# OkDoky/mpc_ros

Measured on AMD Instinct MI355X. Metric: NMPC solves/sec (whole node), N=20 diff-drive, at 1/2/4/8 MI355X, higher is better.
Workload: dtype f64

## Files before the change

### mpc_ros_amd/csrc/mpcg_wide_kern.h

```cpp
#ifndef MPCG_WIDE_KERN_H
#define MPCG_WIDE_KERN_H
#include <hip/hip_runtime.h>

#include "mpcg_internal.h"
#include "mpcg_pp.h"
#include "wave_dev.h"
#include "wide_core.h"
#include "wide_plan.h"

namespace mpcg {


struct WideArgs {
    IpmParams P;
    int64_t B;
    const int32_t* order;
    const double* state;
    const double* coeffs;
    double* u0;
    double* traj;
    int32_t* status;
    double* obj;
    int32_t* iters;
    int32_t* diag;
// ... 70 lines not shown
template <class Solver>
__device__ __forceinline__ void write_out(const WideArgs& a, Solver& S, int64_t p, int parked);
template <bool VHOLD = false>
__device__ __forceinline__ PPRow pp_load_row(const double* pparams, int64_t p) {
    typedef const double __attribute__((address_space(4))) cdouble;
    const cdouble* row = (const cdouble*)(pparams + p * MPCG_PP_FIELDS);
    PPRow r;
#pragma unroll
    for (int j = 0; j < MPCG_PP_FIELDS; ++j) {
        r.f[j] = row[j];
        if constexpr (VHOLD) asm("" : "+v"(r.f[j]));
    }
    return r;
}
#ifndef MPCG_PP_ROW_SGPR
#define MPCG_PP_ROW_SGPR 0
#endif
__device__ __forceinline__ void pp_invalid_out(const WideArgs& a, int64_t p) {
    const int t = threadIdx.x;
    if (t == 0) {
        a.u0[p * 2 + 0] = 0.0;
        a.u0[p * 2 + 1] = 0.0;
        if (a.status) a.status[p] = IPM_INTERNAL_ERROR;
        if (a.iters) a.iters[p] = 0;
        if (a.obj) a.obj[p] = __builtin_nan("");
    }
    if (a.diag && t < 4) a.diag[p * 4 + t] = 0;
    if (a.traj)
        for (int k = t; k < 3 * a.P.N; k += 64) a.traj[p * 3 * a.P.N + k] = 0.0;
    if (a.sol)
        for (int64_t e = t; e < a.sol_stride; e += 64) a.sol[p * a.sol_stride + e] = 0.0;
}

template <int MODEL, bool SPLIT, class T, int NB, bool DEFOPT, bool WARM, bool PP = false>
__device__ __forceinline__ void solve_body(const WideArgs& a, const double* pparams = nullptr) {
    if ((int64_t)blockIdx.x >= a.B) return;
    const int64_t p = a.order ? (int64_t)a.order[blockIdx.x] : (int64_t)blockIdx.x;
    check_index_quiet(p, a.n_prob);
    const int t = threadIdx.x;
    IpmProblem<T> pr;
#pragma unroll
    for (int j = 0; j < 6; ++j) pr.init[j] = (T)a.state[p * 6 + j];
#pragma unroll
    for (int j = 0; j < 4; ++j) pr.c[j] = (T)a.coeffs[p * 4 + j];
    DevWave wv;
    wv.t = t;
    IpmParams Pk = a.P;
    if constexpr (DEFOPT) ipopt_default_options(Pk);
    if (blockIdx.x == 0 && t == 0) atomicExch(a.started, 1);
    if constexpr (PP) {
        const PPRow row = pp_load_row<!MPCG_PP_ROW_SGPR>(pparams, p);
        if (!pp_row_ok(row.f, MODEL)) {
            pp_invalid_out(a, p);
            block_done(a.done);
            return;
        }
        pp_row_apply(row.f, Pk);
    }
    const int slot = claim_slot(a.slot_flags, a.nslots, a.nxcc, (int64_t)blockIdx.x);
    check_index_quiet(slot, a.nslots);
    typedef WideSolver<DevWave, MODEL, SPLIT, T, NB> Solver;
    Solver S(Pk, pr, wv, (T*)a.slots + (int64_t)slot * a.slot_elems);
    if constexpr (WARM) {
        const float* h = a.handoff + p * a.handoff_stride;
        if (__builtin_amdgcn_readfirstlane(h[0] != 0.0f ? 1 : 0))
            S.init_warm(h);
        else
            S.init();
        S.run();
    } else {
        S.solve();
    }
    if constexpr (sizeof(T) == 4) {
        if (a.handoff) {
            S.handoff_out(a.handoff + p * a.handoff_stride);
            release_slot(a.slot_flags, slot);
            block_done(a.done);
            return;
        }
    }
    if (S.status == Solver::NEED_RESTO) {
        int e = 0;
        if (t == 0) e = atomicAdd(a.park_count, 1);
        e = __builtin_amdgcn_readfirstlane(__shfl(e, 0, 64));
        if (e < a.park_cap) {
            check_index_quiet(e, a.park_cap);
            S.park((T*)a.park + (int64_t)e * a.park_stride, p);
            if (t == 0) a.park_idx[e] = p;
            __builtin_amdgcn_fence(__ATOMIC_RELEASE, "agent");
            __builtin_amdgcn_wave_barrier();
            if (t == 0) atomicExch(&a.park_ready[e], 1);
            release_slot(a.slot_flags, slot);
            block_done(a.done);
            return;
        }
        if (t == 0) {
            const int o = atomicAdd(a.ovf_count, 1);
            check_index_quiet(o, a.B);
            atomicExch((unsigned long long*)&a.ovf_idx[o], (unsigned long long)p);
        }
        release_slot(a.slot_flags, slot);
        block_done(a.done);
        return;
    }
    write_out(a, S, p, 0);
    release_slot(a.slot_flags, slot);
    block_done(a.done);
}

template <int MODEL, bool SPLIT, class T, int NB, bool DEFOPT = false, int WPE = 2>
__global__ void __launch_bounds__(64) __attribute__((amdgpu_waves_per_eu(WPE, WPE))) k_solve_wide(WideArgs a) {
    solve_body<MODEL, SPLIT, T, NB, DEFOPT, false>(a);
}
template <int MODEL, bool SPLIT, class T, int NB, bool DEFOPT = false, int WPE = 2>
__global__ void __launch_bounds__(64) __attribute__((amdgpu_waves_per_eu(WPE, WPE))) k_warm_wide(WideArgs a) {
    solve_body<MODEL, SPLIT, T, NB, DEFOPT, true>(a);
}

template <int MODEL, bool SPLIT, class T, int NB, bool DEFOPT = false, int WPE = 2>
__global__ void __launch_bounds__(64) __attribute__((amdgpu_waves_per_eu(WPE, WPE)))
k_solve_wide_pp(WideArgs a, const double* pparams) {
    solve_body<MODEL, SPLIT, T, NB, DEFOPT, false, true>(a, pparams);
}

template <class Solver>
__device__ __forceinline__ void write_out(const WideArgs& a, Solver& S, int64_t p, int parked) {
    const int t = threadIdx.x;
    if (a.diag && t == 0) {
        if (a.handoff && sizeof(typename Solver::T) == 8) parked = a.handoff[p * a.handoff_stride] != 0.0f ? 4 : 3;
        a.diag[p * 4 + 0] = S.n_resto;
        a.diag[p * 4 + 1] = S.n_fover;
        a.diag[p * 4 + 2] = parked;
        a.diag[p * 4 + 3] = S.nf_peak;
#ifdef MPCG_DEBUG_MU
        a.diag[p * 4 + 1] = (int)(-100.0 * log10((double)S.mu));
        a.diag[p * 4 + 3] = (int)(-100.0 * log10((double)S.compl0 + 1e-300));
#endif
    }
    const double o = (double)S.objective_out();
    const int N = a.P.N;
    if (t == 0) {
        a.u0[p * 2 + 0] = (double)S.x_ctrl(0, 0);
        a.u0[p * 2 + 1] = (double)S.x_ctrl(1, 0);
        if (a.status) a.status[p] = S.status;
        if (a.iters) a.iters[p] = S.iter;
// ... 69 lines not shown
                continue;
            }
            if ((int64_t)d >= a.B) break;
            const uint64_t now = wall_clock64();
            if (d == 0 && now - t_start > (uint64_t)200000 &&
                __hip_atomic_load(a.started, __ATOMIC_RELAXED, __HIP_MEMORY_SCOPE_AGENT) == 0)
                break;
            if (d != last_done) {
                last_done = d;
                t0 = now;
            } else if (now - t0 > (uint64_t)2000000000) {
                break;
            }
            __builtin_amdgcn_s_sleep(32);
        }
        if (o >= 0) {
            for (;;) {
                p = (int64_t)__hip_atomic_load((unsigned long long*)&a.ovf_idx[o], __ATOMIC_ACQUIRE,
                                               __HIP_MEMORY_SCOPE_AGENT);
                if (p >= 0) break;
                __builtin_amdgcn_s_sleep(8);
            }
        }
    }
    const int lo = __builtin_amdgcn_readfirstlane(__shfl((int)(p & 0xffffffff), 0, 64));
    const int hi = __builtin_amdgcn_readfirstlane(__shfl((int)(p >> 32), 0, 64));
    return (int64_t)(((uint64_t)(uint32_t)hi << 32) | (uint32_t)lo);
}

template <int MODEL, bool SPLIT, class T, int NB>
__global__ void __launch_bounds__(64) __attribute__((amdgpu_waves_per_eu(1, 1))) k_resume_wide(WideArgs a) {
    const int t = threadIdx.x;
    const WideLayout Lw(a.P.N, a.P.filter_cap, MODEL);
    typedef WideSolver<DevWave, MODEL, SPLIT, T, NB> Solver;
    for (;;) {
        int64_t p;
        T* ent;
        if (a.phase == 0) {
            const int e = take_parked(a);
            if (e < 0) return;
            check_index("parked entry", e, a.park_cap);
            p = a.park_idx[e];
            check_index("parked problem", p, a.n_prob);
            ent = (T*)a.park + (int64_t)e * a.park_stride;
        } else {
            p = take_overflow(a);
            if (p < 0) return;
            check_index("overflow problem", p, a.n_prob);
            check_index("overflow worker's park entry", (int64_t)a.ent0 + blockIdx.x, a.park_cap);
            ent = (T*)a.park + (int64_t)(a.ent0 + blockIdx.x) * a.park_stride;
        }
        IpmProblem<T> pr;
#pragma unroll
        for (int j = 0; j < 6; ++j) pr.init[j] = (T)a.state[p * 6 + j];
#pragma unroll
        for (int j = 0; j < 4; ++j) pr.c[j] = (T)a.coeffs[p * 4 + j];
        DevWave wv;
        wv.t = t;
        Solver S(a.P, pr, wv, ent + Solver::PARK_SCALARS + Lw.total());
        if (a.phase == 0) {
            if (!S.park_entry_ok(ent, p)) index_fault("parked entry's tag / counts: problem", p, a.n_prob);
            S.unpark(ent);
        } else {
            if (a.handoff && a.handoff[p * a.handoff_stride] != 0.0f)
                S.init_warm(a.handoff + p * a.handoff_stride);
            else
                S.init();
            S.run();
        }
        S.finish_resto();
        write_out(a, S, p, a.phase == 0 ? 1 : a.ovf_mark);
    }
}
template <int MODEL, bool SPLIT, class T, int NB>
__global__ void __launch_bounds__(64) __attribute__((amdgpu_waves_per_eu(1, 1)))
k_resume_wide_pp(WideArgs a, const double* pparams) {
    const int t = threadIdx.x;
    const WideLayout Lw(a.P.N, a.P.filter_cap, MODEL);
    typedef WideSolver<DevWave, MODEL, SPLIT, T, NB> Solver;
    for (;;) {
        int64_t p;
        T* ent;
        if (a.phase == 0) {
            const int e = take_parked(a);
            if (e < 0) return;
            check_index("parked entry", e, a.park_cap);
            p = a.park_idx[e];
            check_index("parked problem", p, a.n_prob);
            ent = (T*)a.park + (int64_t)e * a.park_stride;
        } else {
            p = take_overflow(a);
            if (p < 0) return;
            check_index("overflow problem", p, a.n_prob);
            check_index("overflow worker's park entry", (int64_t)a.ent0 + blockIdx.x, a.park_cap);
            ent = (T*)a.park + (int64_t)(a.ent0 + blockIdx.x) * a.park_stride;
        }
        IpmProblem<T> pr;
#pragma unroll
        for (int j = 0; j < 6; ++j) pr.init[j] = (T)a.state[p * 6 + j];
#pragma unroll
        for (int j = 0; j < 4; ++j) pr.c[j] = (T)a.coeffs[p * 4 + j];
        DevWave wv;
        wv.t = t;
        IpmParams Pk = a.P;
        const PPRow row = pp_load_row(pparams, p);
        pp_row_apply(row.f, Pk);
        Solver S(Pk, pr, wv, ent + Solver::PARK_SCALARS + Lw.total());
        if (a.phase == 0) {
            if (!S.park_entry_ok(ent, p)) index_fault("parked entry's tag / counts: problem", p, a.n_prob);
            S.unpark(ent);
        } else {
            S.init();
// ... 43 lines not shown
```

### mpc_ros_amd/csrc/wide_core.h

```cpp
#ifndef MPCG_WIDE_CORE_H
#define MPCG_WIDE_CORE_H

#include "ipm_core.h"

#ifndef MPCG_FUSE
#define MPCG_FUSE 3
#endif

namespace mpcg {

template <class T>
MPCG_HD T opaque(T v) {
#if defined(__HIP_DEVICE_COMPILE__)
    asm volatile("" : "+v"(v));
#endif
    return v;
}

struct WideLayout {
    int N, cap, SS;
    int KL;
    MPCG_HD WideLayout(int N_, int cap_, int model, int kl = -1)
        : N(N_), cap(cap_), SS(model == 1 ? 42 : 38), KL(kl >= 0 ? kl : (model == 1 || N_ > 32 ? 0 : KS)) {}
    static constexpr int WS = 10, YS = 6, KS = 18;
    static constexpr int RS = 34, RZL = 8, RZU = 16, RDW = 24;
    static constexpr int SA = 0;
    static constexpr int SDT = 7;
    static constexpr int SD = 8;
    static constexpr int SQD = 14;
    static constexpr int SQV = 22;
    static constexpr int SCV = 30;
    static constexpr int SZERO = 35, SONE = 36, SMONE = 37;
    static constexpr int KF = 16;
    static constexpr int STW = 38, STV = 39, SHVD = 40;
    MPCG_HD int W(int k) const { return RS * k; }
    MPCG_HD int ZL(int k) const { return RS * k + RZL; }
    MPCG_HD int ZU(int k) const { return RS * k + RZU; }
    MPCG_HD int DW(int k) const { return RS * k + RDW; }
    MPCG_HD int Y(int k) const { return RS * N + YS * k; }
// ... 25 lines not shown
    static constexpr int XM = 48;
    static constexpr int XMN = 84;
    static constexpr int XMV = 120;
    static constexpr int XE = 126;
    static constexpr int XRX = 132, XRP = 140, XRN = 146, XRC = 152;
    static constexpr int XSX = 158, XSP = 166, XSN = 172, XSY = 178, XSC = 184;
    static constexpr int XS = 190;
    static constexpr int XW = 72;
    MPCG_HD int SP_DUMP() const { return spill(); }
    MPCG_HD int SP_EXT() const { return spill() + total(); }
    MPCG_HD int SP_XSP() const { return SP_EXT() + XS * N; }
    MPCG_HD int SP_FLTR() const { return SP_XSP() + XW * N; }
    MPCG_HD int slot() const { return SP_FLTR() + 2 * FX; }
    static constexpr int PARK_SCALARS = 32, HANDOFF_HEAD = 4;
    MPCG_HD int park() const { return PARK_SCALARS + total() + slot(); }
    MPCG_HD static int handoff(int N_) { return HANDOFF_HEAD + 30 * N_; }
};

MPCG_HD int64_t solution_elems(int N) { return 3 * (int64_t)(8 * N - 2) + 6 * (int64_t)N; }

template <class T>
struct RestoIn {
    T mu, tau, theta, prim_inf, ref_phi, ref_theta, sf;
    int nf, iter;
};
struct RestoOut {
    int status;
    int iter;
    int fover;
};
template <class WV, int MODEL, class T, int NB>
MPCG_NOINLINE RestoOut resto_phase(const IpmParams& P, IpmProblem<T> pr, WV wv, T* ws, RestoIn<T> in);

template <class WV, int MODEL = 0, bool SPLIT = false, class TT = double, int NB = 1, bool RESTO = false>
struct WideSolver {
    static_assert(NB == 1 || !SPLIT, "the half-wave split is for N <= 32");
    static_assert(!RESTO || !SPLIT, "the restoration problem runs the unsplit sweeps");
    typedef TT T;
    static constexpr double EPS = sizeof(TT) == 4 ? 1.1920928955078125e-07 : 2.220446049250313e-16;
    const IpmParams P;
    const IpmProblem<T> pr;
    WV wv;
    WideLayout L;
    int N, t;
    T dt;
    T sl, su, wl, wu, al, au, sl0, su0, wl0, wu0, al0, au0;
    T sf;
    T mu, tau;
    T fval, logsum, theta, prim_inf, prim_uns, dual_inf, compl0, pmin, pmax, l1y, l1z;
    T theta_min, dw_last, acc_alpha, acc_z, delta_w_used;
    int iter, nf, status;
    bool acc_pending;
    T ref_theta, ref_phi, ref_gd, ref_pgd, ref_pth, ref_inc;
    int last_rej_filter, count_filter_rej, n_filter_resets;
    int in_wd, wd_short, wd_trial_iter, tiny_last, tiny_flag, in_soft, soft_count, acc_counter, have_acc;

    T* spill;
    int n_fover = 0;
    int nf_peak = 0;
    int n_resto = 0;
    struct CtlRef {
        const WideSolver* s;
        int i;
        MPCG_HD operator T() const { return s->wv.uni_d(s->ld(s->L.CTL() + i)); }
        MPCG_HD CtlRef& operator=(T v) {
            s->wv.sync();
            if (s->wv.lane() == 0) s->st(s->L.CTL() + i, v);
            s->wv.sync();
            return *this;
        }
        MPCG_HD CtlRef& operator=(const CtlRef& o) { return *this = (T)o; }
    };
    MPCG_HD CtlRef wd_alpha_test() const { return CtlRef{this, 0}; }
    MPCG_HD CtlRef wd_theta() const { return CtlRef{this, 1}; }
    MPCG_HD CtlRef wd_phi() const { return CtlRef{this, 2}; }
    MPCG_HD CtlRef wd_gd() const { return CtlRef{this, 3}; }
    MPCG_HD CtlRef wd_amax_z() const { return CtlRef{this, 4}; }
    MPCG_HD CtlRef soc_alpha() const { return CtlRef{this, 5}; }
    MPCG_HD CtlRef soc_amax_z() const { return CtlRef{this, 6}; }
    MPCG_HD CtlRef soc_theta_old() const { return CtlRef{this, 7}; }
    MPCG_HD CtlRef soc_theta_trial() const { return CtlRef{this, 8}; }
    MPCG_HD CtlRef soft_ec() const { return CtlRef{this, 9}; }
    MPCG_HD CtlRef soft_a() const { return CtlRef{this, 10}; }
    MPCG_HD CtlRef last_obj() const { return CtlRef{this, 11}; }
    MPCG_HD CtlRef curr_obj() const { return CtlRef{this, 12}; }
    MPCG_HD CtlRef kkt() const { return CtlRef{this, 13}; }
    MPCG_HD CtlRef theta_max() const { return CtlRef{this, 14}; }
    MPCG_HD CtlRef last_mu() const { return CtlRef{this, 15}; }

    T c_sa = 0, c_ca = 0;
    int c_ok = 0;
    static constexpr bool FUSE_SQ = SPLIT && sizeof(TT) == 8 && (MPCG_FUSE & 1) != 0;
    static constexpr bool FUSE_RED = SPLIT && sizeof(TT) == 8 && (MPCG_FUSE & 2) != 0;
    int sq_ok = 0;
    MPCG_HD void sq_drop() {
        if constexpr (FUSE_SQ) sq_ok = 0;
    }
    static constexpr int model = MODEL;
    T lf;

    static constexpr double RHO = 1000.0;
    static constexpr double KD = 1e-5;
    enum : int { RESTO_DONE = 100 };
    enum : int { NEED_RESTO = 101 };
    T* ext = nullptr;
    T* xsp = nullptr;
    T* dumpO = nullptr;
    T o_mu = 0, o_tau = 0, o_theta = 0, o_ref_phi = 0, o_ref_theta = 0, o_sf = 1;
    int o_nf = 0;
    bool resto_first = false;
    T r_spn = 0, r_qx = 0, r_phiO = 0, r_thO = 0, r_pinfO = 0;
    bool rf_pass = false;
    T mu_Emu = 0;
    int mu_tf = 0;
    bool mu_done = false;

    MPCG_HD WideSolver(const IpmParams& P_, const IpmProblem<T>& pr_, const WV& wv_, T* spill_)
        : P(P_), pr(pr_), wv(wv_), L(P_.N, P_.filter_cap, MODEL, MODEL == 0 && SPLIT ? WideLayout::KS : -1), N(P_.N), t(wv_.t), dt((T)P_.dt), lf((T)P_.lf),
          spill(spill_) {}

    MPCG_HD void next_m(const Lin<T>& ln, const T* s, const T* u, T* out) const {
        ln.next(s, u, dt, out);
        if (model == 1) {
            const T turn = s[3] * u[0] / lf * dt;
            out[2] = s[2] + turn;
            out[5] = s[5] + turn;
        }
    }
    MPCG_HD void turn_d(const T* s, const T* u, T* tw, T* tv) const {
        if (model == 1) {
// ... 227 lines not shown
                }
                if (j < 6) {
                    const T y = ld(L.Y(k) + j), yp = ld(L.YP(k) + j);
                    st(L.Y(k) + j, y + alpha * (yp - y));
                }
            }
            if constexpr (RESTO) accept_rows(t, alpha, amax_z, clamp);
        }
        wv.sync();
    }
    MPCG_HD void accept_rows(int t, T alpha, T amax_z, bool clamp) {
        for (int b = 0; b < NB; ++b) {
            const int k = t + 64 * b;
            if (k >= N) continue;
            T* x = xrec(k);
#pragma unroll
            for (int j = 0; j < 6; ++j) {
#pragma unroll
                for (int h = 0; h < 2; ++h) {
                    const int ov = h ? WideLayout::XN : WideLayout::XP, oz = h ? WideLayout::XZN : WideLayout::XZP;
                    const int od = h ? WideLayout::XDN : WideLayout::XDP;
                    const T v = x[ov + j], z = x[oz + j], dv = x[od + j];
                    const T dz = mu / v - z - z / v * dv;
                    const T vn = v + alpha * dv;
                    T zn = z + amax_z * dz;
                    if (clamp) zn = tmax(tmin(zn, (T)1e10 * mu / vn), mu / ((T)1e10 * vn));
                    x[ov + j] = vn;
                    x[oz + j] = zn;
                }
            }
        }
    }

    MPCG_HD void stats_split(bool acc, T alpha, T amax_z) {
        const int t = wv.lane();
        accept_all(t, acc, alpha, amax_z);
        wv.mark(16);
        const bool reuse = acc && c_ok;
        c_ok = 0;
        const bool sums_known = FUSE_RED && reuse;
        const int k = t & 31;
        const bool hi = t >= 32, act = k < N, last = k == N - 1;
        const int j0 = hi ? 4 : 0, nr = hi ? 2 : 4;
        const int sbk = L.ST(k);
        T sqd[4] = {0, 0, 0, 0}, sqv[4] = {0, 0, 0, 0};
        T f = 0, th = 0, pinf = 0, puns = 0, dinf = 0, mn = (T)INFINITY, mx = -(T)INFINITY, ly = 0, lz = 0,
          lg = 0;
        T Fa[4] = {0, 0, 0, 0}, A[4] = {0, 0, 0, 0};
        T w[8], zl[4], zu[4], yq[4], yn[6] = {0, 0, 0, 0, 0, 0}, up[2] = {0, 0}, um[2] = {0, 0};
        T twk = dt, tvk = 0, f1 = 0;
        if (act) {
            ldn<8>(L.W(k), w);
            ldv<4>(L.ZL(k) + j0, zl);
            ldv<4>(L.ZU(k) + j0, zu);
            ldv<4>(L.Y(k) + j0, yq);
            const int sb = L.ST(k);
            T cv[3] = {0, 0, 0};
            if (!last) {
                ldn<6>(L.Y(k + 1), yn);
                up[0] = ld(L.W(k + 1) + 6);
                up[1] = ld(L.W(k + 1) + 7);
                T sa, ca;
                if (reuse) {
                    sa = c_sa;
                    ca = c_ca;
                } else {
                    sc_t(hi ? w[5] : w[2], &sa, &ca);
                }
                const T x = w[0], v = w[3];
                const C4 pcoef_ = pcoef();
                const T fx = pcoef_.c[0] + pcoef_.c[1] * x + pcoef_.c[2] * (x * x) + pcoef_.c[3] * (x * x * x);
                f1 = pcoef_.c[1] + (T)2 * pcoef_.c[2] * x + (T)3 * pcoef_.c[3] * x * x;
                const T f2 = (T)2 * pcoef_.c[2] + (T)6 * pcoef_.c[3] * x;
                A[0] = hi ? f1 : -w[3] * sa * dt;
                A[1] = hi ? sa * dt : ca * dt;
                A[2] = w[3] * ca * dt;
                A[3] = sa * dt;
                T turn = w[6] * dt;
                if (model == 1) turn = w[3] * w[6] / lf * dt;
                Fa[0] = (hi ? fx - w[1] : w[0]) + w[3] * (hi ? sa : ca) * dt;
                Fa[1] = hi ? (model == 1 ? w[5] + turn : w[5] + w[6] * dt) : w[1] + w[3] * sa * dt;
                Fa[2] = model == 1 ? w[2] + turn : w[2] + w[6] * dt;
                Fa[3] = w[3] + w[7] * dt;
                turn_d(w, w + 6, &twk, &tvk);
                cv[0] = hi ? -yn[4] * f2 : yn[0] * v * ca * dt + yn[1] * v * sa * dt;
                cv[1] = hi ? yn[4] * v * sa * dt : yn[0] * sa * dt - yn[1] * ca * dt;
                cv[2] = -yn[4] * ca * dt;
                T wn[4];
// ... 63 lines not shown
            if (!sums_known) {
                const T e1 = w[4] - (T)P.ref_cte, e2 = w[5] - (T)P.ref_eth, e3 = w[3] - (T)P.ref_v;
                T fu = (T)P.w_cte * e1 * e1 + (T)P.w_eth * e2 * e2;
                if (!last) fu += cost_ctrl(k, w + 6, up);
                f = hi ? fu : (T)P.w_v * e3 * e3;
            }
            const T btw = twk * (yn[2] + yn[5]), bta = dt * yn[3];
            const T g3 = (T)(2.0 * P.w_v) * (w[3] - (T)P.ref_v);
            const T g4 = (T)(2.0 * P.w_cte) * (w[4] - (T)P.ref_cte), g5 = (T)(2.0 * P.w_eth) * (w[5] - (T)P.ref_eth);
            const int nv = (last && hi) ? 2 : 4;
            T slackprod = 1;
#pragma unroll
            for (int q = 0; q < 4; ++q) {
                if (q < nv) {
                    const T wq = hi ? w[4 + q] : w[q];
                    T gj;
                    if (q < 2)
                        gj = hi ? sf * (q == 0 ? g4 : g5) + yq[q] - at[q] : sf * (T)0 + yq[q] - at[q];
                    else
                        gj = hi ? sf * gu[q - 2] - (q == 2 ? btw : bta) : (q == 2 ? sf * (T)0 : sf * g3) + yq[q] - at[q];
                    const T rd = gj - zl[q] + zu[q];
                    dinf = tmax(dinf, (T)fabs(rd));
                    const T lo = q < 2 ? sl : (q == 2 ? (hi ? wl : sl) : (hi ? al : sl));
                    const T hb = q < 2 ? su : (q == 2 ? (hi ? wu : su) : (hi ? au : su));
                    const T dl = wq - lo, du = hb - wq;
                    if (!sums_known) slackprod *= dl * du;
                    const T p1 = dl * zl[q], p2 = du * zu[q];
                    mn = tmin(mn, tmin(p1, p2));
                    mx = tmax(mx, tmax(p1, p2));
                    lz += fabs(zl[q]) + fabs(zu[q]);
                    if constexpr (FUSE_SQ) {
                        const T gq = opaque(hi ? (q == 0 ? g4 : (q == 1 ? g5 : gu[q - 2])) : (q == 3 ? g3 : (T)0));
                        const T hq = hi ? (q < 2 ? hess_state(4 + q) : hess_ctrl(k, q - 2)) : hess_state(q);
                        sq_terms(hq, gq, wq - lo, hb - wq, zl[q], zu[q], &sqd[q], &sqv[q]);
                    }
                }
            }
            if (!sums_known) lg = log(slackprod);
            if constexpr (FUSE_SQ) {
#pragma unroll
                for (int q = 0; q < 4; ++q) {
                    st(sbk + WideLayout::SQD + j0 + q, sqd[q]);
                    st(sbk + WideLayout::SQV + j0 + q, sqv[q]);
                }
            }
        }
        if constexpr (FUSE_SQ) sq_ok = 1;
        if (sums_known) {
            T v[7] = {pinf, puns, dinf, mn, mx, ly, lz};
            const int op[7] = {RMAX, RMAX, RMAX, RMIN, RMAX, RSUM, RSUM};
            reduce<7, true>(v, op);
            fval = tr_f;
            theta = tr_theta;
            prim_inf = v[0];
            prim_uns = v[1];
            dual_inf = v[2];
            pmin = v[3];
            pmax = v[4];
            l1y = v[5];
            l1z = v[6];
            logsum = tr_lg;
        } else {
            T v[10] = {f, th, pinf, puns, dinf, mn, mx, ly, lz, lg};
            const int op[10] = {RSUM, RSUM, RMAX, RMAX, RMAX, RMIN, RMAX, RSUM, RSUM, RSUM};
            reduce<10, true>(v, op);
            fval = v[0];
            theta = v[1];
            prim_inf = v[2];
            prim_uns = v[3];
            dual_inf = v[4];
            pmin = v[5];
            pmax = v[6];
            l1y = v[7];
            l1z = v[8];
            logsum = v[9];
        }
        compl0 = wv.uni_d(tmax(pmax, -pmin));
        wv.mark(0);
    }

// ... 307 lines not shown
            f += cost_state(w);
            if (!last) {
                T up[2];
                up[0] = ld(L.W(k + 1) + 6) + alpha * ld(L.DW(k + 1) + 6);
                up[1] = ld(L.W(k + 1) + 7) + alpha * ld(L.DW(k + 1) + 7);
                f += cost_ctrl(k, w + 6, up);
                Lin<T> ln;
                ln.eval(pcoef().c, w);
                next_m(ln, w, w + 6, Fk[b]);
            }
        }
        T Fprev[NB][6];
        shift_blocks(Fk, Fprev);
        for (int b = 0; b < NB; ++b) {
            const int k = t + 64 * b;
            if (k >= N) continue;
#pragma unroll
            for (int j = 0; j < 6; ++j) {
                const T wj = ld(L.W(k) + j) + alpha * ld(L.DW(k) + j);
                const T c = k == 0 ? wj - pinit(j) : wj - Fprev[b][j];
                thv += fabs(rowscale(j, k) * c);
            }
        }
        T v[3] = {f, thv, lg};
        const int op[3] = {RSUM, RSUM, RSUM};
        reduce<3, true>(v, op);
        const bool anybad = wv.any(bad != 0);
        wv.mark(6);
        *phi = sf * v[0] - mu * v[2];
        *th = v[1];
        return !anybad && isfinite((double)*phi);
    }

    MPCG_HD void sq_terms(T hq, T gq, T dl, T du, T zl, T zu, T* qd, T* qv) const {
        const T rdl = rcp(dl), rdu = rcp(du);
        *qd = sf * hq + zl * rdl + zu * rdu;
        *qv = sf * gq - mu * rdl + mu * rdu;
    }
    MPCG_HD void precompute_split(int mode, T delta_w) {
        const int t = wv.lane();
        const int k = t & 31;
        const bool hi = t >= 32;
        if (k >= N) return;
        const bool last = k == N - 1;
        const int sb = L.ST(k);
        if (mode == 1 && !hi) {
            T w[8];
            ldn<8>(L.W(k), w);
            T a[7] = {0, 0, 0, 0, 0, 0, 0}, tw = dt, tv = 0;
            if (!last) {
                Lin<T> ln;
                ln.eval(pcoef().c, w);
                ln.jac(w, dt, a);
                turn_d(w, w + 6, &tw, &tv);
            }
#pragma unroll
            for (int j = 0; j < 7; ++j) st(sb + WideLayout::SA + j, a[j]);
            if constexpr (MODEL == 1) {
                st(sb + WideLayout::STW, tw);
                st(sb + WideLayout::STV, tv);
                st(sb + WideLayout::SHVD, 0);
            }
#pragma unroll
            for (int j = 0; j < 6; ++j) st(sb + WideLayout::SD + j, 0);
#pragma unroll
            for (int j = 0; j < 5; ++j) st(sb + WideLayout::SCV + j, 0);
        }
        const int j0 = hi ? 4 : 0;
        T w[4], zl[4], zu[4];
        ldv<4>(L.W(k) + j0, w);
        ldv<4>(L.ZL(k) + j0, zl);
        ldv<4>(L.ZU(k) + j0, zu);
        T gu[2] = {0, 0};
        if (!last) {
            T um[2] = {0, 0}, up[2];
            if (k >= 1) {
                um[0] = ld(L.W(k - 1) + 6);
                um[1] = ld(L.W(k - 1) + 7);
            }
            up[0] = ld(L.W(k + 1) + 6);
            up[1] = ld(L.W(k + 1) + 7);
            grad_ctrl(k, um, w + 2, up, gu);
        }
        const T g3 = (T)(2.0 * P.w_v) * (w[3] - (T)P.ref_v);
        const T g4 = (T)(2.0 * P.w_cte) * (w[0] - (T)P.ref_cte), g5 = (T)(2.0 * P.w_eth) * (w[1] - (T)P.ref_eth);
        const int nv = (last && hi) ? 2 : 4;
#pragma unroll
        for (int q = 0; q < 4; ++q) {
            T qd = 0, qv = 0;
            if (q < nv) {
                const T gq = hi ? (q == 0 ? g4 : (q == 1 ? g5 : gu[q - 2])) : (q == 3 ? g3 : (T)0);
                const T hq = hi ? (q < 2 ? hess_state(4 + q) : hess_ctrl(k, q - 2)) : hess_state(q);
                const T lo = q < 2 ? sl : (q == 2 ? (hi ? wl : sl) : (hi ? al : sl));
                const T hb = q < 2 ? su : (q == 2 ? (hi ? wu : su) : (hi ? au : su));
                if (mode == 0) {
                    sq_terms(hq, gq, w[q] - lo, hb - w[q], zl[q], zu[q], &qd, &qv);
                    qd += delta_w;
                } else {
                    qd = 1;
                    qv = sf * gq - zl[q] + zu[q];
                }
            }
            st(sb + WideLayout::SQD + j0 + q, qd);
            st(sb + WideLayout::SQV + j0 + q, qv);
        }
    }

    MPCG_HD void precompute(int mode, T delta_w) {
        if constexpr (RESTO) {
            const int t = wv.lane();
            for (int b = 0; b < NB; ++b) precompute_resto(t + 64 * b, delta_w);
            wv.gsync();
            return;
        }
        if constexpr (SPLIT) {
            precompute_split(mode, delta_w);
            return;
        }
        const int t = wv.lane();
        if constexpr (NB == 2) {
            precompute_stage(t, mode, delta_w);
            precompute_stage(t + 64, mode, delta_w);
            return;
        }
        precompute_stage(t, mode, delta_w);
    }
    MPCG_HD void precompute_stage(int k, int mode, T delta_w) {
        if (k >= N) return;
        const bool last = k == N - 1;
// ... 235 lines not shown
        F.amax_z = tmin(F.amax_z, dzl < 0 ? -tau * zl * rcp(dzl) : inf);
        F.amax_z = tmin(F.amax_z, dzu < 0 ? -tau * zu * rcp(dzu) : inf);
        F.gd += gphi * dwv;
        F.rel = tmax(F.rel, (T)fabs(dwv) * rcp((T)1 + (T)fabs(w)));
    }

    MPCG_HD void step_stats_split(int k, const T* xk, const T* duk, Fwd& F) const {
        const int t = wv.lane();
        const bool hi = t >= 32, last = k == N - 1;
        const int j0 = hi ? 4 : 0;
        T w[4], zl[4], zu[4];
        ldv<4>(L.W(k) + j0, w);
        ldv<4>(L.ZL(k) + j0, zl);
        ldv<4>(L.ZU(k) + j0, zu);
        T gu[2] = {0, 0};
        if (!last) {
            T um[2] = {0, 0}, up[2];
            if (k >= 1) {
                um[0] = ld(L.W(k - 1) + 6);
                um[1] = ld(L.W(k - 1) + 7);
            }
            up[0] = ld(L.W(k + 1) + 6);
            up[1] = ld(L.W(k + 1) + 7);
            const T u[2] = {w[2], w[3]};
            grad_ctrl(k, um, u, up, gu);
        }
        const T g4 = (T)(2.0 * P.w_cte) * (w[0] - (T)P.ref_cte), g5 = (T)(2.0 * P.w_eth) * (w[1] - (T)P.ref_eth);
        const T g3 = (T)(2.0 * P.w_v) * (w[3] - (T)P.ref_v);
        const T gq[4] = {hi ? sf * g4 : sf * (T)0, hi ? sf * g5 : sf * (T)0, hi ? sf * gu[0] : sf * (T)0,
                         hi ? sf * gu[1] : sf * g3};
        const T dq[4] = {hi ? xk[4] : xk[0], hi ? xk[5] : xk[1], hi ? duk[0] : xk[2], hi ? duk[1] : xk[3]};
        const T lo2 = hi ? wl : sl, hi2 = hi ? wu : su, lo3 = hi ? al : sl, hi3 = hi ? au : su;
        const int nv = (last && hi) ? 2 : 4;
#pragma unroll
        for (int q = 0; q < 4; ++q) {
            if (q < nv) {
                const T lo = q < 2 ? sl : (q == 2 ? lo2 : lo3), up_ = q < 2 ? su : (q == 2 ? hi2 : hi3);
                const T rdl = rcp(w[q] - lo), rdu = rcp(up_ - w[q]);
                const T gphi = gq[q] - mu * rdl + mu * rdu;
                dir_var_r(w[q], zl[q], zu[q], lo, up_, gphi, dq[q], rdl, rdu, F);
            }
        }
    }

    MPCG_HD bool kr_hbm() const {
        if constexpr (MODEL == 0 && SPLIT)
            return false;
        else
            return L.KL == 0;
    }
    MPCG_HD void ld_gains(int k, T* K, T* kf) const {
        if (kr_hbm()) {
            const T* g = spill + L.SP_KRG() + WideLayout::KS * k;
#pragma unroll
            for (int q = 0; q < 16; ++q) K[q] = g[q];
            kf[0] = g[WideLayout::KF];
            kf[1] = g[WideLayout::KF + 1];
        } else {
            ldv<16>(L.KR(k), K);
            ldv<2>(L.KR(k) + WideLayout::KF, kf);
        }
    }
    MPCG_HD void forward_begin() const {
        wv.sync();
        if (kr_hbm()) wv.gsync();
    }

    MPCG_HD Fwd forward(int mode) {
        if constexpr (RESTO) return forward_resto();
        if constexpr (NB == 2) return forward_blk(mode);
        const int t = wv.lane();
// ... 85 lines not shown
                    tva = ld(sb + WideLayout::STV);
                    hvd = ld(sb + WideLayout::SHVD);
                }
                const T* x = xk;
                base[0] = (qd[0] + cv[0]) * x[0] + qv[0];
                base[1] = qd[1] * x[1] + qv[1];
                base[2] = (qd[2] + cv[1]) * x[2] + cv[2] * x[3] + qv[2];
                base[3] = qd[3] * x[3] + cv[2] * x[2] + cv[4] * x[5] + qv[3];
                base[4] = qd[4] * x[4] + qv[4];
                base[5] = (qd[5] + cv[3]) * x[5] + cv[4] * x[3] + qv[5];
                if constexpr (MODEL == 1) base[3] += hvd * duk[0];
            } else {
#pragma unroll
                for (int q = 0; q < 8; ++q) ak[q] = 0;
            }
        }
#pragma unroll
        for (int q = 0; q < 6; ++q) lam[q] = 0;
        T o[6];
        for (int s = N - 1; s >= 0; --s) {
            AT_mul(ak, lam, o);
            if constexpr (MODEL == 1) o[3] += tva * (lam[2] + lam[5]);
#pragma unroll
            for (int q = 0; q < 6; ++q) o[q] += base[q];
            wv.dn6(lam, o);
        }
        if (t < N) {
#pragma unroll
            for (int q = 0; q < 6; ++q) st(L.YP(t) + q, -o[q]);
        }
        wv.mark(4);
        Fwd F{(T)1, (T)1, (T)0, (T)0};
        if constexpr (SPLIT) {
            if (mode == 0 && ks < N) step_stats_split(ks, xk, duk, F);
        } else if (t < N) {
            const int k = t;
            const bool last = k == N - 1;
            if (mode == 0) {
                T w[8], zl[8], zu[8], dk[8];
                ldn<8>(L.W(k), w);
                ldn<8>(L.ZL(k), zl);
                ldn<8>(L.ZU(k), zu);
#pragma unroll
                for (int q = 0; q < 6; ++q) dk[q] = xk[q];
                dk[6] = duk[0];
                dk[7] = duk[1];
                T g[6], gu[2] = {0, 0};
                grad_state(w, g);
                if (!last) {
                    T um[2] = {0, 0}, up[2];
                    if (k >= 1) {
                        um[0] = ld(L.W(k - 1) + 6);
                        um[1] = ld(L.W(k - 1) + 7);
                    }
                    up[0] = ld(L.W(k + 1) + 6);
                    up[1] = ld(L.W(k + 1) + 7);
                    grad_ctrl(k, um, w + 6, up, gu);
                }
                const int nv = last ? 6 : 8;
#pragma unroll
                for (int j = 0; j < 8; ++j) {
                    if (j < nv) {
                        const T gj = j < 6 ? sf * g[j] : sf * gu[j - 6];
                        const T gphi = gj - mu * rcp(w[j] - vlo(j)) + mu * rcp(vhi(j) - w[j]);
                        dir_var(w[j], zl[j], zu[j], vlo(j), vhi(j), gphi, dk[j], F);
                    }
// ... 1665 lines not shown

    MPCG_HD int set_op(int o, int c) {
        op = o;
        ct = c;
        return LS_CONT;
    }
    MPCG_HD int do_trial(T alpha, T alpha_test, int c) {
        tr_alpha = wv.uni_d(alpha);
        tr_test = wv.uni_d(alpha_test);
        return set_op(OP_TRIAL, c);
    }
    MPCG_HD int do_solve(int mode, T delta, int c) {
        sv_mode = mode;
        sv_delta = wv.uni_d(delta);
        return set_op(OP_SOLVE, c);
    }
    MPCG_HD int do_stats(bool acc, T alpha, T z, int c) {
        st_acc = acc;
        st_alpha = alpha;
        st_z = z;
        return set_op(OP_STATS, c);
    }

    MPCG_HD void init() {
        setup();
        init_point();
        reset_state((T)P.mu_init, 0);
        do_solve(1, (T)0, K_LSQ);
    }
    MPCG_HD void reset_state(T mu0, int it0) {
        mu = wv.uni_d(mu0);
        tau = wv.uni_d(tmax((T)0.99, (T)1 - mu0));
        status = 0;
        sq_drop();
        theta_max() = -1;
        theta_min = -1;
        dw_last = 0;
        delta_w_used = 0;
        acc_alpha = 0;
        acc_z = 0;
        acc_pending = false;
        iter = it0;
        nf = 0;
        kkt() = 0;
        ref_theta = ref_phi = ref_gd = ref_pgd = ref_pth = 0;
        last_rej_filter = count_filter_rej = n_filter_resets = 0;
        in_wd = wd_short = wd_trial_iter = tiny_last = tiny_flag = in_soft = soft_count = acc_counter = have_acc = 0;
        wd_alpha_test() = wd_theta() = wd_phi() = wd_gd() = wd_amax_z() = 0;
        last_mu() = -1;
        last_obj() = 0;
        curr_obj() = (T)-1e50;
        cur_acceptable = false;
        st_acc = sv_ok = tr_ok = false;
        st_alpha = st_z = tr_alpha = tr_test = tr_phi = tr_theta = pd_val = 0;
        tr_acc = false;
        ls_alpha = ls_alpha_max = ls_alpha_min = ls_alpha_test = ls_amax_z = 0;
        ls_n_steps = inertia_attempt = soft_ctx = 0;
        ls_eval_error = ls_skip_first = wd_from_tiny = false;
        soc_alpha() = soc_amax_z() = soc_theta_old() = soc_theta_trial() = soft_ec() = soft_a() = 0;
        soc_count = 0;
        lsF = Fwd{(T)1, (T)1, (T)0, (T)0};
        sv_F = lsF;
    }

    static constexpr int HANDOFF_HEAD = WideLayout::HANDOFF_HEAD;
    MPCG_HD static int handoff_elems(int N_) { return WideLayout::handoff(N_); }
    MPCG_HD void handoff_out(float* h) const {
// ... 288 lines not shown
    }
    MPCG_HD int bt_done(bool accept) {
        if (in_wd) {
            if (accept) {
                in_wd = 0;
                return ls_finish(true, false);
            }
            ++wd_trial_iter;
            if (ls_eval_error || wd_trial_iter > P.watchdog_trial_max) {
                wd_from_tiny = false;
                return stop_watchdog();
            }
            return ls_finish(true, false);
        }
        return ls_finish(accept, false);
    }
    MPCG_HD void start_watchdog(const Fwd& F) {
        in_wd = 1;
        spill_out(L.SP_WD(), 0, (WideLayout::RS + 2 * WideLayout::YS) * N);
        xcopy(true, WideLayout::XP, 0, 36);
        wd_trial_iter = 0;
        wd_alpha_test() = F.amax_p;
        wd_amax_z() = F.amax_z;
        wd_theta() = ref_theta;
        wd_phi() = ref_phi;
        wd_gd() = ref_gd;
    }
    MPCG_HD int stop_watchdog() {
        in_wd = 0;
        spill_in(L.SP_WD(), 0, (WideLayout::RS + 2 * WideLayout::YS) * N);
        xcopy(false, WideLayout::XP, 0, 36);
        wd_short = 0;
        c_ok = 0;
        sq_drop();
        return do_stats(false, (T)0, (T)0, K_WD_STATS);
    }
    MPCG_HD int k_wd_stats() {
        set_ref(wd_theta(), wd_phi(), wd_gd());
        lsF.amax_p = wd_alpha_test();
        lsF.amax_z = wd_amax_z();
        lsF.gd = wd_gd();
        ls_skip_first = !wd_from_tiny;
        return bt_start();
    }

    MPCG_HD int soft_start() {
        soft_a() = wv.uni_d(tmin(lsF.amax_p, lsF.amax_z));
        return do_trial(soft_a(), (T)0, K_SOFT_TRIAL);
    }
    MPCG_HD int k_soft_trial() {
        if (!tr_ok) return soft_done(false, false);
        if (tr_acc) {
            acc_alpha = soft_a();
            acc_z = soft_a();
            acc_pending = true;
            return soft_done(true, true);
        }
        return set_op(OP_PDERR, K_SOFT_PD0);
    }
    MPCG_HD int k_soft_pd0() {
        soft_ec() = pd_val;
        rec_out<0, 24>(L.SP_SOFT());
        spill_out(L.SP_SOFT() + 3 * WideLayout::WS * N, L.Y(0), WideLayout::YS * N);
        xcopy(true, WideLayout::XP, 48, 24);
        accept_all(wv.lane(), true, soft_a(), soft_a(), false);
        c_ok = 0;
        sq_drop();
        return set_op(OP_PDERR, K_SOFT_PD1);
    }
    MPCG_HD int k_soft_pd1() {
        if (wv.uni(pd_val <= (T)P.soft_resto_factor * soft_ec())) {
            clamp_all();
            return soft_done(true, false);
        }
        rec_in<0, 24>(L.SP_SOFT());
        spill_in(L.SP_SOFT() + 3 * WideLayout::WS * N, L.Y(0), WideLayout::YS * N);
        xcopy(false, WideLayout::XP, 48, 24);
        return soft_done(false, false);
    }
    MPCG_HD int soft_done(bool accept, bool sat) {
        if (soft_ctx == 0) {
            if (accept && sat) {
                in_soft = 0;
                soft_count = 0;
            }
            return accept ? ls_done() : ls_fail();
        }
        if (accept) {
            in_soft = !sat;
            return ls_done();
        }
        return ls_fail();
    }

    MPCG_HD int ls_finish(bool accept, bool soft_or_resto) {
        if (!accept) {
            if (!in_soft && P.soft_resto_factor > 0) {
                augment_filter();
                soft_ctx = 1;
                return soft_start();
            }
            return ls_fail();
        }
        if (!soft_or_resto) {
            acc_alpha = wv.uni_d(ls_alpha);
            acc_z = wv.uni_d(ls_amax_z);
            acc_pending = true;
            if (ls_n_steps == 0)
                wd_short = 0;
            else
                ++wd_short;
        }
        return ls_done();
    }
    MPCG_HD int ls_done() {
        wv.mark(7);
        ++iter;
        return do_stats(acc_pending, acc_alpha, acc_z, K_BEGIN);
    }
    MPCG_HD int ls_fail() {
        if (!in_soft) augment_filter();
        if constexpr (RESTO) {
            return IPM_RESTORATION_FAILURE;
        } else {
            if (wv.uni(theta <= (T)1e-2 * (T)P.tol)) {
                if (have_acc) {
                    rec_in<0, 8>(L.SP_ACC());
                    sq_drop();
                    return IPM_ACCEPTABLE;
                }
                return IPM_RESTORATION_FAILURE;
            }
            if (P.no_resto) return IPM_RESTORATION_FAILURE;
            in_soft = 0;
            soft_count = 0;
            wd_short = 0;
            return NEED_RESTO;
        }
    }
    MPCG_HD int ls_goto_resto() {
        if (mu != last_mu()) {
            in_wd = 0;
            wd_short = 0;
            last_mu() = mu;
        }
        if (P.acceptable_iter > 0 && cur_acceptable) {
            rec_out<0, 8>(L.SP_ACC());
            have_acc = 1;
        }
        if (in_wd) {
            wd_from_tiny = true;
            return stop_watchdog();
        }
        return ls_fail();
    }
    MPCG_HD int restoration() {
        ++n_resto;
        spill_out(L.SP_DUMP(), 0, L.total());
        wv.gsync();
        const RestoIn<T> in{mu, tau, theta, prim_inf, ref_phi, ref_theta, sf, nf, iter};
        const IpmParams Pc = P;
        const RestoOut o = resto_phase<WV, MODEL, T, NB>(Pc, pr, wv, spill, in);
        wv.gsync();
        spill_in(L.SP_DUMP(), 0, L.total());
        iter = wv.uni(o.iter);
        n_fover += wv.uni(o.fover);
        c_ok = 0;
        sq_drop();
        const int s = wv.uni(o.status);
        if (s) return s;
        clamp_all();
        acc_pending = false;
        ++iter;
        return do_stats(false, (T)0, (T)0, K_BEGIN);
    }

    MPCG_HD RestoOut run_resto(const RestoIn<T>& in) {
        dumpO = spill + L.SP_DUMP();
        ext = spill + L.SP_EXT();
        xsp = spill + L.SP_XSP();
        bounds_only();
        sf = wv.uni_d((T)1);
        o_mu = wv.uni_d(in.mu);
        o_tau = wv.uni_d(in.tau);
        o_theta = wv.uni_d(in.theta);
        o_ref_phi = wv.uni_d(in.ref_phi);
        o_ref_theta = wv.uni_d(in.ref_theta);
        o_sf = wv.uni_d(in.sf);
        o_nf = wv.uni(in.nf);
        mu = wv.uni_d(tmax(in.mu, in.prim_inf));
        tau = wv.uni_d(tmax((T)0.99, (T)1 - mu));
        status = 0;
        theta_max() = -1;
        theta_min = -1;
        dw_last = 0;
        delta_w_used = 0;
        acc_alpha = 0;
        acc_z = 0;
        acc_pending = false;
        iter = wv.uni(in.iter);
        nf = 0;
// ... 241 lines not shown
        wv.sync();
        const T* img = src + PARK_SCALARS;
        for (int e = t; e < L.total(); e += 64) st(e, img[e]);
        wv.sync();
        mu = wv.uni_d(src[0]);
        tau = wv.uni_d(src[1]);
        theta = wv.uni_d(src[2]);
        prim_inf = wv.uni_d(src[3]);
        ref_phi = wv.uni_d(src[4]);
        ref_theta = wv.uni_d(src[5]);
        sf = wv.uni_d(src[6]);
        theta_min = wv.uni_d(src[7]);
        dw_last = wv.uni_d(src[8]);
        delta_w_used = wv.uni_d(src[9]);
        iter = wv.uni((int)src[10]);
        nf = wv.uni((int)src[11]);
        last_rej_filter = wv.uni((int)src[12]);
        count_filter_rej = wv.uni((int)src[13]);
        n_filter_resets = wv.uni((int)src[14]);
        tiny_last = wv.uni((int)src[15]);
        tiny_flag = wv.uni((int)src[16]);
        acc_counter = wv.uni((int)src[17]);
        have_acc = wv.uni((int)src[18]);
        in_wd = wv.uni((int)src[19]);
        wd_short = wv.uni((int)src[20]);
        in_soft = wv.uni((int)src[21]);
        soft_count = wv.uni((int)src[22]);
        wd_trial_iter = wv.uni((int)src[23]);
        n_fover = wv.uni((int)src[24]);
        n_resto = wv.uni((int)src[25]);
        nf_peak = wv.uni((int)src[26]);
        status = NEED_RESTO;
        c_ok = 0;
        sq_drop();
        acc_pending = false;
        cur_acceptable = false;
    }
    MPCG_HD void run() {
        for (;;) {
            const int o = wv.uni(op);
            if (o == OP_STATS) {
                stats(st_acc, st_alpha, st_z);
            } else if (o == OP_SOLVE) {
                sv_ok = wv.uni(riccati(sv_mode, sv_delta));
                if (sv_ok) sv_F = forward(sv_mode);
                if constexpr (RESTO) {
                    if (sv_ok) sv_F = refine_resto();
                }
            } else if (o == OP_TRIAL) {
                tr_ok = trial(tr_alpha, &tr_phi, &tr_theta);
                tr_acc = tr_ok && check_acceptability(tr_test, tr_phi, tr_theta);
                wv.mark(10);
            } else if (o == OP_PDERR) {
                pd_val = pd_error();
            } else {
                soc_rhs(soc_alpha());
            }
            const int s = step(wv.uni(ct));
            wv.mark(13);
            if (s > 0) {
                status = s;
                break;
            }
        }
        wv.sync();
    }

// ... 55 lines not shown
```

Baseline: 4.297 million.

## Cache barrier reciprocals in registers and fuse step acceptance into split stats

Adds per-lane register storage for the lower and upper barrier reciprocals 1/(w-lo) and 1/(hi-w). These are reused across stats, the condensed-Hessian terms and step-direction recovery instead of being recomputed. A fused accept path updates w, z and y, keeps the new values in registers for the stats pass, and avoids reloading them from the workspace. The path is enabled only for the split f64 default-options diff-drive kernel at 2 waves per EU. It costs extra VGPRs and adds invalidation points that must stay correct across resto, watchdog and soft-restoration paths.

```diff
diff --git a/mpc_ros_amd/csrc/mpcg_wide_kern.h b/mpc_ros_amd/csrc/mpcg_wide_kern.h
--- a/mpc_ros_amd/csrc/mpcg_wide_kern.h
+++ b/mpc_ros_amd/csrc/mpcg_wide_kern.h
@@ -126,7 +126,7 @@
         for (int64_t e = t; e < a.sol_stride; e += 64) a.sol[p * a.sol_stride + e] = 0.0;
 }
 
-template <int MODEL, bool SPLIT, class T, int NB, bool DEFOPT, bool WARM, bool PP = false>
+template <int MODEL, bool SPLIT, class T, int NB, bool DEFOPT, bool WARM, bool PP = false, bool RCK = false>
 __device__ __forceinline__ void solve_body(const WideArgs& a, const double* pparams = nullptr) {
     if ((int64_t)blockIdx.x >= a.B) return;
     const int64_t p = a.order ? (int64_t)a.order[blockIdx.x] : (int64_t)blockIdx.x;
@@ -153,7 +153,7 @@
     }
     const int slot = claim_slot(a.slot_flags, a.nslots, a.nxcc, (int64_t)blockIdx.x);
     check_index_quiet(slot, a.nslots);
-    typedef WideSolver<DevWave, MODEL, SPLIT, T, NB> Solver;
+    typedef WideSolver<DevWave, MODEL, SPLIT, T, NB, false, RCK> Solver;
     Solver S(Pk, pr, wv, (T*)a.slots + (int64_t)slot * a.slot_elems);
     if constexpr (WARM) {
         const float* h = a.handoff + p * a.handoff_stride;
@@ -204,7 +204,7 @@
 
 template <int MODEL, bool SPLIT, class T, int NB, bool DEFOPT = false, int WPE = 2>
 __global__ void __launch_bounds__(64) __attribute__((amdgpu_waves_per_eu(WPE, WPE))) k_solve_wide(WideArgs a) {
-    solve_body<MODEL, SPLIT, T, NB, DEFOPT, false>(a);
+    solve_body<MODEL, SPLIT, T, NB, DEFOPT, false, false, DEFOPT && MODEL == 0 && WPE == 2>(a);
 }
 template <int MODEL, bool SPLIT, class T, int NB, bool DEFOPT = false, int WPE = 2>
 __global__ void __launch_bounds__(64) __attribute__((amdgpu_waves_per_eu(WPE, WPE))) k_warm_wide(WideArgs a) {
@@ -340,7 +340,7 @@
 __global__ void __launch_bounds__(64) __attribute__((amdgpu_waves_per_eu(1, 1))) k_resume_wide(WideArgs a) {
     const int t = threadIdx.x;
     const WideLayout Lw(a.P.N, a.P.filter_cap, MODEL);
-    typedef WideSolver<DevWave, MODEL, SPLIT, T, NB> Solver;
+    typedef WideSolver<DevWave, MODEL, SPLIT, T, NB, false, false> Solver;
     for (;;) {
         int64_t p;
         T* ent;
@@ -385,7 +385,7 @@
 k_resume_wide_pp(WideArgs a, const double* pparams) {
     const int t = threadIdx.x;
     const WideLayout Lw(a.P.N, a.P.filter_cap, MODEL);
-    typedef WideSolver<DevWave, MODEL, SPLIT, T, NB> Solver;
+    typedef WideSolver<DevWave, MODEL, SPLIT, T, NB, false, false> Solver;
     for (;;) {
         int64_t p;
         T* ent;
diff --git a/mpc_ros_amd/csrc/wide_core.h b/mpc_ros_amd/csrc/wide_core.h
--- a/mpc_ros_amd/csrc/wide_core.h
+++ b/mpc_ros_amd/csrc/wide_core.h
@@ -4,7 +4,7 @@
 #include "ipm_core.h"
 
 #ifndef MPCG_FUSE
-#define MPCG_FUSE 3
+#define MPCG_FUSE 15
 #endif
 
 namespace mpcg {
@@ -96,8 +96,21 @@
 template <class WV, int MODEL, class T, int NB>
 MPCG_NOINLINE RestoOut resto_phase(const IpmParams& P, IpmProblem<T> pr, WV wv, T* ws, RestoIn<T> in);
 
-template <class WV, int MODEL = 0, bool SPLIT = false, class TT = double, int NB = 1, bool RESTO = false>
-struct WideSolver {
+template <class T, bool ON>
+struct RcRegs {
+    T rc_l[4] = {0, 0, 0, 0}, rc_u[4] = {0, 0, 0, 0};
+    int rc_ok = 0;
+};
+template <class T>
+struct RcRegs<T, false> {};
+template <bool SPLIT, class T, bool RCK>
+constexpr bool wide_fuse_rc() {
+    return SPLIT && sizeof(T) == 8 && RCK && (MPCG_FUSE & 5) == 5;
+}
+
+template <class WV, int MODEL = 0, bool SPLIT = false, class TT = double, int NB = 1, bool RESTO = false,
+          bool RCK = true>
+struct WideSolver : RcRegs<TT, wide_fuse_rc<SPLIT, TT, RCK>()> {
     static_assert(NB == 1 || !SPLIT, "the half-wave split is for N <= 32");
     static_assert(!RESTO || !SPLIT, "the restoration problem runs the unsplit sweeps");
     typedef TT T;
@@ -160,6 +173,21 @@
     MPCG_HD void sq_drop() {
         if constexpr (FUSE_SQ) sq_ok = 0;
     }
+    static constexpr bool FUSE_RC = wide_fuse_rc<SPLIT, TT, RCK>();
+    static constexpr bool FUSE_AC = FUSE_RC && (MPCG_FUSE & 8) != 0;
+    MPCG_HD void rc_drop() {
+        if constexpr (FUSE_RC) this->rc_ok = 0;
+    }
+    MPCG_HD bool rc_held() const {
+        if constexpr (FUSE_RC)
+            return this->rc_ok != 0;
+        else
+            return false;
+    }
+    MPCG_HD void iter_drop() {
+        sq_drop();
+        rc_drop();
+    }
     static constexpr int model = MODEL;
     T lf;
 
@@ -453,10 +481,81 @@
         }
     }
 
+    MPCG_HD void accept_split(bool acc, T alpha, T amax_z, T* zlo, T* zuo, T* yo) {
+        const int t = wv.lane();
+        wv.sync();
+        if constexpr (FUSE_AC) {
+            if (acc) {
+                const bool have = wv.uni(rc_held());
+                const int k = t & 31;
+                const bool hi = t >= 32, last = k == N - 1;
+                if (k < N) {
+                    const int j0 = hi ? 4 : 0, nv = (last && hi) ? 2 : 4, nr = hi ? 2 : 4;
+                    T w[4], dw[4], zl[4], zu[4];
+                    ldv<4>(L.W(k) + j0, w);
+                    ldv<4>(L.DW(k) + j0, dw);
+                    ldv<4>(L.ZL(k) + j0, zl);
+                    ldv<4>(L.ZU(k) + j0, zu);
+#pragma unroll
+                    for (int q = 0; q < 4; ++q) {
+                        if (q < nv) {
+                            const T lo = q < 2 ? sl : (q == 2 ? (hi ? wl : sl) : (hi ? al : sl));
+                            const T hb = q < 2 ? su : (q == 2 ? (hi ? wu : su) : (hi ? au : su));
+                            T rdl, rdu;
+                            if (have) {
+                                rdl = opaque(this->rc_l[q]);
+                                rdu = opaque(this->rc_u[q]);
+                            } else {
+                                rdl = rcp(w[q] - lo);
+                                rdu = rcp(hb - w[q]);
+                            }
+                            const T dzl = mu * rdl - zl[q] - zl[q] * rdl * dw[q];
+                            const T dzu = mu * rdu - zu[q] + zu[q] * rdu * dw[q];
+                            const T wn = w[q] + alpha * dw[q];
+                            const T a = zl[q] + amax_z * dzl, b = zu[q] + amax_z * dzu;
+                            const T ksig = (T)1e10, iksig = (T)1e-10;
+                            const T rs2 = rcp(wn - lo), ru2 = rcp(hb - wn);
+                            zl[q] = tmax(tmin(a, ksig * mu * rs2), mu * rs2 * iksig);
+                            zu[q] = tmax(tmin(b, ksig * mu * ru2), mu * ru2 * iksig);
+                            w[q] = wn;
+                            this->rc_l[q] = rs2;
+                            this->rc_u[q] = ru2;
+                        }
+                    }
+#pragma unroll
+                    for (int q = 0; q < 4; ++q) {
+                        st(L.W(k) + j0 + q, w[q]);
+                        st(L.ZL(k) + j0 + q, zl[q]);
+                        st(L.ZU(k) + j0 + q, zu[q]);
+                    }
+                    T y[4], yp[4];
+                    ldv<4>(L.Y(k) + j0, y);
+                    ldv<4>(L.YP(k) + j0, yp);
+#pragma unroll
+                    for (int q = 0; q < 4; ++q) {
+                        if (q < nr) {
+                            y[q] = y[q] + alpha * (yp[q] - y[q]);
+                            st(L.Y(k) + j0 + q, y[q]);
+                        }
+                        zlo[q] = zl[q];
+                        zuo[q] = zu[q];
+                        yo[q] = y[q];
+                    }
+                }
+                this->rc_ok = 1;
+            }
+        }
+        wv.sync();
+    }
+
     MPCG_HD void stats_split(bool acc, T alpha, T amax_z) {
         const int t = wv.lane();
-        accept_all(t, acc, alpha, amax_z);
-        wv.mark(16);
+        T azl[4] = {0, 0, 0, 0}, azu[4] = {0, 0, 0, 0}, ay[4] = {0, 0, 0, 0};
+        if constexpr (FUSE_AC)
+            accept_split(acc, alpha, amax_z, azl, azu, ay);
+        else
+            accept_all(t, acc, alpha, amax_z);
+        wv.mark(FUSE_AC && acc ? 21 : 16);
         const bool reuse = acc && c_ok;
         c_ok = 0;
         const bool sums_known = FUSE_RED && reuse;
@@ -472,9 +571,18 @@
         T twk = dt, tvk = 0, f1 = 0;
         if (act) {
             ldn<8>(L.W(k), w);
-            ldv<4>(L.ZL(k) + j0, zl);
-            ldv<4>(L.ZU(k) + j0, zu);
-            ldv<4>(L.Y(k) + j0, yq);
+            if (FUSE_AC && acc) {
+#pragma unroll
+                for (int q = 0; q < 4; ++q) {
+                    zl[q] = azl[q];
+                    zu[q] = azu[q];
+                    yq[q] = ay[q];
+                }
+            } else {
+                ldv<4>(L.ZL(k) + j0, zl);
+                ldv<4>(L.ZU(k) + j0, zu);
+                ldv<4>(L.Y(k) + j0, yq);
+            }
             const int sb = L.ST(k);
             T cv[3] = {0, 0, 0};
             if (!last) {
@@ -604,7 +712,22 @@
                     if constexpr (FUSE_SQ) {
                         const T gq = opaque(hi ? (q == 0 ? g4 : (q == 1 ? g5 : gu[q - 2])) : (q == 3 ? g3 : (T)0));
                         const T hq = hi ? (q < 2 ? hess_state(4 + q) : hess_ctrl(k, q - 2)) : hess_state(q);
-                        sq_terms(hq, gq, wq - lo, hb - wq, zl[q], zu[q], &sqd[q], &sqv[q]);
+                        bool took = false;
+                        if constexpr (FUSE_AC) {
+                            if (acc) {
+                                sq_terms_r(hq, gq, opaque(this->rc_l[q]), opaque(this->rc_u[q]), zl[q], zu[q], &sqd[q],
+                                           &sqv[q]);
+                                took = true;
+                            }
+                        }
+                        if (!took) {
+                            T rl, ru;
+                            sq_terms(hq, gq, wq - lo, hb - wq, zl[q], zu[q], &sqd[q], &sqv[q], &rl, &ru);
+                            if constexpr (FUSE_RC) {
+                                this->rc_l[q] = rl;
+                                this->rc_u[q] = ru;
+                            }
+                        }
                     }
                 }
             }
@@ -618,6 +741,7 @@
             }
         }
         if constexpr (FUSE_SQ) sq_ok = 1;
+        if constexpr (FUSE_RC) this->rc_ok = 1;
         if (sums_known) {
             T v[7] = {pinf, puns, dinf, mn, mx, ly, lz};
             const int op[7] = {RMAX, RMAX, RMAX, RMIN, RMAX, RSUM, RSUM};
@@ -991,8 +1115,13 @@
         return !anybad && isfinite((double)*phi);
     }
 
-    MPCG_HD void sq_terms(T hq, T gq, T dl, T du, T zl, T zu, T* qd, T* qv) const {
+    MPCG_HD void sq_terms(T hq, T gq, T dl, T du, T zl, T zu, T* qd, T* qv, T* rl, T* ru) const {
         const T rdl = rcp(dl), rdu = rcp(du);
+        sq_terms_r(hq, gq, rdl, rdu, zl, zu, qd, qv);
+        *rl = rdl;
+        *ru = rdu;
+    }
+    MPCG_HD void sq_terms_r(T hq, T gq, T rdl, T rdu, T zl, T zu, T* qd, T* qv) const {
         *qd = sf * hq + zl * rdl + zu * rdu;
         *qv = sf * gq - mu * rdl + mu * rdu;
     }
@@ -1053,7 +1182,8 @@
                 const T lo = q < 2 ? sl : (q == 2 ? (hi ? wl : sl) : (hi ? al : sl));
                 const T hb = q < 2 ? su : (q == 2 ? (hi ? wu : su) : (hi ? au : su));
                 if (mode == 0) {
-                    sq_terms(hq, gq, w[q] - lo, hb - w[q], zl[q], zu[q], &qd, &qv);
+                    T rl, ru;
+                    sq_terms(hq, gq, w[q] - lo, hb - w[q], zl[q], zu[q], &qd, &qv, &rl, &ru);
                     qd += delta_w;
                 } else {
                     qd = 1;
@@ -1355,11 +1485,24 @@
         const T dq[4] = {hi ? xk[4] : xk[0], hi ? xk[5] : xk[1], hi ? duk[0] : xk[2], hi ? duk[1] : xk[3]};
         const T lo2 = hi ? wl : sl, hi2 = hi ? wu : su, lo3 = hi ? al : sl, hi3 = hi ? au : su;
         const int nv = (last && hi) ? 2 : 4;
+        const bool rc_have = FUSE_RC && wv.uni(rc_held());
 #pragma unroll
         for (int q = 0; q < 4; ++q) {
             if (q < nv) {
                 const T lo = q < 2 ? sl : (q == 2 ? lo2 : lo3), up_ = q < 2 ? su : (q == 2 ? hi2 : hi3);
-                const T rdl = rcp(w[q] - lo), rdu = rcp(up_ - w[q]);
+                T rdl, rdu;
+                bool took = false;
+                if constexpr (FUSE_RC) {
+                    if (rc_have) {
+                        rdl = this->rc_l[q];
+                        rdu = this->rc_u[q];
+                        took = true;
+                    }
+                }
+                if (!took) {
+                    rdl = rcp(w[q] - lo);
+                    rdu = rcp(up_ - w[q]);
+                }
                 const T gphi = gq[q] - mu * rdl + mu * rdu;
                 dir_var_r(w[q], zl[q], zu[q], lo, up_, gphi, dq[q], rdl, rdu, F);
             }
@@ -1511,6 +1654,7 @@
         wv.mark(4);
         Fwd F{(T)1, (T)1, (T)0, (T)0};
         if constexpr (SPLIT) {
+            wv.mark(mode != 0 ? 20 : (rc_held() ? 18 : 19));
             if (mode == 0 && ks < N) step_stats_split(ks, xk, duk, F);
         } else if (t < N) {
             const int k = t;
@@ -3242,7 +3386,7 @@
         mu = wv.uni_d(mu0);
         tau = wv.uni_d(tmax((T)0.99, (T)1 - mu0));
         status = 0;
-        sq_drop();
+        iter_drop();
         theta_max() = -1;
         theta_min = -1;
         dw_last = 0;
@@ -3597,7 +3741,7 @@
         xcopy(false, WideLayout::XP, 0, 36);
         wd_short = 0;
         c_ok = 0;
-        sq_drop();
+        iter_drop();
         return do_stats(false, (T)0, (T)0, K_WD_STATS);
     }
     MPCG_HD int k_wd_stats() {
@@ -3630,7 +3774,7 @@
         xcopy(true, WideLayout::XP, 48, 24);
         accept_all(wv.lane(), true, soft_a(), soft_a(), false);
         c_ok = 0;
-        sq_drop();
+        iter_drop();
         return set_op(OP_PDERR, K_SOFT_PD1);
     }
     MPCG_HD int k_soft_pd1() {
@@ -3641,6 +3785,7 @@
         rec_in<0, 24>(L.SP_SOFT());
         spill_in(L.SP_SOFT() + 3 * WideLayout::WS * N, L.Y(0), WideLayout::YS * N);
         xcopy(false, WideLayout::XP, 48, 24);
+        iter_drop();
         return soft_done(false, false);
     }
     MPCG_HD int soft_done(bool accept, bool sat) {
@@ -3691,7 +3836,7 @@
             if (wv.uni(theta <= (T)1e-2 * (T)P.tol)) {
                 if (have_acc) {
                     rec_in<0, 8>(L.SP_ACC());
-                    sq_drop();
+                    iter_drop();
                     return IPM_ACCEPTABLE;
                 }
                 return IPM_RESTORATION_FAILURE;
@@ -3731,7 +3876,7 @@
         iter = wv.uni(o.iter);
         n_fover += wv.uni(o.fover);
         c_ok = 0;
-        sq_drop();
+        iter_drop();
         const int s = wv.uni(o.status);
         if (s) return s;
         clamp_all();
@@ -4039,7 +4184,7 @@
         nf_peak = wv.uni((int)src[26]);
         status = NEED_RESTO;
         c_ok = 0;
-        sq_drop();
+        iter_drop();
         acc_pending = false;
         cur_acceptable = false;
     }
```

After: 4.352 million, median of 6. +1.3%, better.
